# MoFHeka/MeepoEmbedding

Hardware: AMD Instinct MI355X
Metric: key-lookups/sec (higher is better)
Workload: dtype int64 keys / fp32 rows (copy)

## Files before the change

### meepoembedding_amd/csrc/meepo_router.hip

```cpp
#include <hip/hip_runtime.h>

#include <cstdlib>
#include <cstring>
#include <new>

#include "meepo_device.h"
#include "meepo_host.h"

struct mee_router {
    int device;
    uint64_t max_batch;
    uint32_t n_shards;
    uint32_t max_blocks;
    uint32_t* blockcnt;
    uint64_t* base;
    uint64_t* run_base;
    uint64_t* run_sums;
};

struct mee_p2p {
    int device;
    uint32_t n_shards, rank, dim;
    uint64_t cap, max_batch;
    int64_t* inbox_keys;
    int32_t* inbox_dst;
    uint32_t* inbox_cnt;
    float* out;
    uint8_t* found;
    float* inbox_rows;
    uint32_t* status;
    void** d_tables;
    void* h_tables[6][64];
    bool connected;
};

namespace mee {

constexpr int kPartBlock = 1024;
constexpr int kMaxShards = 64;
constexpr uint32_t kNoOwner = 0xFFFFFFFFu;

template <class T>
__device__ __forceinline__ T wave_scan_inclusive(T v, int lane) {
#pragma unroll
    for (int d = 1; d < 64; d <<= 1) {
        const T t = __shfl_up(v, d);
        if (lane >= d) v += t;
    }
    return v;
}

template <bool RANK>
__device__ __forceinline__ uint32_t count_owners(uint32_t o, uint32_t g, uint32_t (&wcnt)[kPartBlock / 64][kMaxShards]) {
    const int lane = threadIdx.x & 63, w = threadIdx.x >> 6;
    uint32_t r = 0;
    for (uint32_t p = 0; p < g; ++p) {
        const uint64_t m = __ballot(o == p);
        if (RANK && o == p) r = (uint32_t)__popcll(m & ((1ull << lane) - 1));
        if (lane == 0) wcnt[w][p] = (uint32_t)__popcll(m);
    }
    __syncthreads();
    if (RANK && o != kNoOwner)
        for (int ww = 0; ww < w; ++ww) r += wcnt[ww][o];
    return r;
}
__device__ __forceinline__ void store_block_counts(const uint32_t (&wcnt)[kPartBlock / 64][kMaxShards], uint32_t g, uint32_t* blockcnt) {
    if (threadIdx.x < g) {
        uint32_t c = 0;
#pragma unroll
        for (int ww = 0; ww < kPartBlock / 64; ++ww) c += wcnt[ww][threadIdx.x];
        blockcnt[(uint64_t)blockIdx.x * g + threadIdx.x] = c;
    }
}

__global__ void hash_batch_kernel(const int64_t* __restrict__ keys, uint64_t n, uint64_t nb, uint32_t g, uint64_t* mix_out,
                                  uint64_t* bucket_out, uint32_t* owner_out) {
    for (uint64_t i = blockIdx.x * (uint64_t)blockDim.x + threadIdx.x; i < n; i += (uint64_t)gridDim.x * blockDim.x) {
        const int64_t k = keys[i];
        if (mix_out) mix_out[i] = mix64((uint64_t)k);
        if (bucket_out) bucket_out[i] = bucket_of(k, nb);
        if (owner_out) owner_out[i] = owner_of(k, g);
    }
}

template <bool SKIP_PAD>
__global__ __launch_bounds__(kPartBlock) void part_count_kernel(const int64_t* __restrict__ keys, uint32_t n, uint32_t g,
                                                                uint32_t* blockcnt) {
    __shared__ uint32_t wcnt[kPartBlock / 64][kMaxShards];
    const uint32_t i = blockIdx.x * kPartBlock + threadIdx.x;
    const int64_t key = i < n ? keys[i] : kEmpty;
    const bool inb = i < n && !(SKIP_PAD && key == kEmpty);
    count_owners<false>(inb ? owner_of(key, g) : kNoOwner, g, wcnt);
    store_block_counts(wcnt, g, blockcnt);
}

__global__ __launch_bounds__(1024) void part_scan_kernel(uint32_t* blockcnt, uint32_t n_blocks, uint32_t g, uint64_t* base,
                                                         uint64_t* counts_out) {
    __shared__ uint64_t total[kMaxShards];
    const int lane = threadIdx.x & 63, w = threadIdx.x >> 6, nw = blockDim.x >> 6;
    for (uint32_t p = w; p < g; p += nw) {
        uint32_t run = 0;
        for (uint32_t b0 = 0; b0 < n_blocks; b0 += 64) {
            const uint32_t b = b0 + lane;
            const uint32_t c = b < n_blocks ? blockcnt[(uint64_t)b * g + p] : 0;
            const uint32_t incl = wave_scan_inclusive(c, lane);
            if (b < n_blocks) blockcnt[(uint64_t)b * g + p] = run + incl - c;
            run += __shfl(incl, 63);
        }
        if (lane == 0) total[p] = run;
    }
    __syncthreads();
    if (threadIdx.x == 0) {
        uint64_t acc = 0;
        for (uint32_t p = 0; p < g; ++p) {
            base[p] = acc;
            counts_out[p] = total[p];
            acc += total[p];
        }
    }
}

template <bool SKIP_PAD>
__global__ __launch_bounds__(kPartBlock) void part_scatter_kernel(const int64_t* __restrict__ keys, uint32_t n, uint32_t g,
                                                                  const uint32_t* __restrict__ blockoff,
                                                                  const uint64_t* __restrict__ base, int64_t* send_keys,
                                                                  int64_t* perm) {
    __shared__ uint32_t wcnt[kPartBlock / 64][kMaxShards];
    const uint32_t i = blockIdx.x * kPartBlock + threadIdx.x;
    const int64_t key = i < n ? keys[i] : kEmpty;
    const bool inb = i < n && !(SKIP_PAD && key == kEmpty);
    const uint32_t o = inb ? owner_of(key, g) : kNoOwner;
    const uint32_t r = count_owners<true>(o, g, wcnt);
    if (inb) {
        const uint64_t dst = base[o] + blockoff[(uint64_t)blockIdx.x * g + o] + r;
        send_keys[dst] = key;
        perm[dst] = (int64_t)i;
    }
}

template <typename T, bool SCATTER>
__global__ void permute_rows_kernel(const T* __restrict__ rows, const int64_t* __restrict__ perm, uint64_t n, uint32_t epr,
                                    T* __restrict__ out) {
    const uint64_t total = n * epr;
    for (uint64_t idx = blockIdx.x * (uint64_t)blockDim.x + threadIdx.x; idx < total; idx += (uint64_t)gridDim.x * blockDim.x) {
        const uint64_t q = idx / epr;
        const uint32_t e = (uint32_t)(idx - q * epr);
        const uint64_t p = (uint64_t)perm[q];
        if (SCATTER) out[p * epr + e] = rows[idx];
        else out[idx] = rows[p * epr + e];
    }
}

template <bool SCATTER>
static int permute_rows(const void* d_rows, const int64_t* d_perm, size_t n, size_t row_bytes, void* d_out, void* stream,
                        const char* name) {
    if (n && (!d_rows || !d_perm || !d_out)) return fail(MEE_ERR_INVALID_ARG, "%s: null argument", name);
    if (n == 0 || row_bytes == 0) return MEE_OK;
    hipStream_t st = (hipStream_t)stream;
    const bool a16 = row_bytes % 16 == 0 && ((uintptr_t)d_rows % 16 == 0) && ((uintptr_t)d_out % 16 == 0);
    const bool a4 = row_bytes % 4 == 0 && ((uintptr_t)d_rows % 4 == 0) && ((uintptr_t)d_out % 4 == 0);
    if (a16) {
        const uint32_t epr = (uint32_t)(row_bytes / 16);
        permute_rows_kernel<float4, SCATTER><<<grid_for(n * epr, 256, 1u << 16), 256, 0, st>>>((const float4*)d_rows, d_perm, n, epr, (float4*)d_out);
    } else if (a4) {
        const uint32_t epr = (uint32_t)(row_bytes / 4);
        permute_rows_kernel<uint32_t, SCATTER><<<grid_for(n * epr, 256, 1u << 16), 256, 0, st>>>((const uint32_t*)d_rows, d_perm, n, epr, (uint32_t*)d_out);
    } else {
        const uint32_t epr = (uint32_t)row_bytes;
        permute_rows_kernel<uint8_t, SCATTER><<<grid_for(n * epr, 256, 1u << 16), 256, 0, st>>>((const uint8_t*)d_rows, d_perm, n, epr, (uint8_t*)d_out);
    }
    MEE_HIP(hipGetLastError());
    return MEE_OK;
}

__device__ __forceinline__ uint32_t last_not_above(const uint64_t* __restrict__ off, uint32_t m, uint64_t i) {
    uint32_t lo = 0, hi = m - 1;
    while (lo < hi) {
        const uint32_t mid = lo + (hi - lo + 1) / 2;
        if (off[mid] <= i) lo = mid; else hi = mid - 1;
    }
    return lo;
}

struct RunPos {
    bool head;
    uint32_t seg;
    uint32_t bag;
    uint32_t seg_end;
};

__device__ __forceinline__ RunPos run_position(const int64_t* __restrict__ perm, const uint64_t* __restrict__ counts, uint32_t g, uint32_t n,
                                               const uint64_t* __restrict__ off, uint32_t n_bags, uint32_t* s_end, uint32_t* s_bag) {
    if (threadIdx.x == 0) {
        uint64_t acc = 0;
        for (uint32_t p = 0; p < g; ++p) {
            const uint64_t c = counts[p];
            acc += c < n ? c : n;
            acc = acc < n ? acc : n;
            s_end[p] = (uint32_t)acc;
        }
    }
    __syncthreads();
    const uint32_t q = blockIdx.x * kPartBlock + threadIdx.x;
    const bool inb = q < s_end[g - 1];
    uint32_t seg = 0;
    while (seg + 1 < g && s_end[seg] <= q) ++seg;
    const uint32_t seg_begin = seg ? s_end[seg - 1] : 0;
    const uint32_t bag = inb ? last_not_above(off, n_bags, (uint64_t)perm[q]) : 0;
    s_bag[threadIdx.x] = bag;
    __syncthreads();
    uint32_t prev = 0;
    if (inb && q > seg_begin) prev = threadIdx.x ? s_bag[threadIdx.x - 1] : last_not_above(off, n_bags, (uint64_t)perm[q - 1]);
    RunPos r;
    r.head = inb && (q == seg_begin || bag != prev);
    r.seg = r.head ? seg : kNoOwner;
    r.bag = bag;
    r.seg_end = s_end[seg];
    return r;
}

__global__ __launch_bounds__(kPartBlock) void run_count_kernel(const int64_t* __restrict__ perm, const uint64_t* __restrict__ counts, uint32_t g, uint32_t n,
                                                              const uint64_t* __restrict__ off, uint32_t n_bags, uint32_t* blockcnt) {
    __shared__ uint32_t s_end[kMaxShards], s_bag[kPartBlock], wcnt[kPartBlock / 64][kMaxShards];
    const RunPos r = run_position(perm, counts, g, n, off, n_bags, s_end, s_bag);
    count_owners<false>(r.seg, g, wcnt);
    store_block_counts(wcnt, g, blockcnt);
}

__global__ __launch_bounds__(kPartBlock) void run_scatter_kernel(const int64_t* __restrict__ perm, const uint64_t* __restrict__ counts, uint32_t g, uint32_t n,
                                                                const uint64_t* __restrict__ off, uint32_t n_bags, const uint32_t* __restrict__ blockoff,
                                                                const uint64_t* __restrict__ run_base, uint32_t* __restrict__ run_bag,
                                                                uint32_t* __restrict__ run_len) {
    __shared__ uint32_t s_end[kMaxShards], s_bag[kPartBlock], wcnt[kPartBlock / 64][kMaxShards];
    const RunPos r = run_position(perm, counts, g, n, off, n_bags, s_end, s_bag);
    const uint32_t rank = count_owners<true>(r.seg, g, wcnt);
    if (r.head) {
        const uint64_t dst = run_base[r.seg] + blockoff[(uint64_t)blockIdx.x * g + r.seg] + rank;
        const uint32_t q = blockIdx.x * kPartBlock + threadIdx.x;
        const uint64_t bag_end = off[r.bag + 1];
        uint32_t lo = q + 1, hi = r.seg_end;
        while (lo < hi) {
            const uint32_t mid = lo + (hi - lo) / 2;
            if ((uint64_t)perm[mid] < bag_end) lo = mid + 1; else hi = mid;
        }
        run_bag[dst] = r.bag;
        run_len[dst] = lo - q;
    }
}

__device__ __forceinline__ uint64_t block_scan_exclusive(uint64_t v, uint64_t* s_w, uint64_t& total) {
    const int lane = threadIdx.x & 63, w = threadIdx.x >> 6, nw = blockDim.x >> 6;
    const uint64_t incl = wave_scan_inclusive(v, lane);
    if (lane == 63) s_w[w] = incl;
    __syncthreads();
    uint64_t before = 0;
    total = 0;
    for (int ww = 0; ww < nw; ++ww) {
        if (ww < w) before += s_w[ww];
        total += s_w[ww];
    }
    __syncthreads();
    return before + incl - v;
}

__global__ __launch_bounds__(kPartBlock) void run_len_sum_kernel(const uint32_t* __restrict__ run_len, uint64_t n_runs, uint64_t* __restrict__ sums) {
    __shared__ uint64_t s_w[kPartBlock / 64];
    const uint64_t i = (uint64_t)blockIdx.x * kPartBlock + threadIdx.x;
    uint64_t total;
    (void)block_scan_exclusive(i < n_runs ? run_len[i] : 0, s_w, total);
    if (threadIdx.x == 0) sums[blockIdx.x] = total;
}

__global__ __launch_bounds__(kPartBlock) void run_len_scan_kernel(uint64_t* sums, uint32_t n_blocks) {
    __shared__ uint64_t s_w[kPartBlock / 64];
    uint64_t carry = 0;
    for (uint32_t b0 = 0; b0 < n_blocks; b0 += kPartBlock) {
        const uint32_t b = b0 + threadIdx.x;
        uint64_t total;
        const uint64_t ex = block_scan_exclusive(b < n_blocks ? sums[b] : 0, s_w, total);
        if (b < n_blocks) sums[b] = carry + ex;
        carry += total;
    }
}

__global__ __launch_bounds__(kPartBlock) void run_offsets_kernel(const uint32_t* __restrict__ run_len, uint64_t n_runs, const uint64_t* __restrict__ sums,
                                                                uint64_t* __restrict__ offsets) {
    __shared__ uint64_t s_w[kPartBlock / 64];
    const uint64_t i = (uint64_t)blockIdx.x * kPartBlock + threadIdx.x;
    const uint64_t len = i < n_runs ? run_len[i] : 0;
    uint64_t total;
    const uint64_t ex = sums[blockIdx.x] + block_scan_exclusive(len, s_w, total);
    if (i < n_runs) offsets[i] = ex;
    if (i + 1 == n_runs) offsets[n_runs] = ex + len;
}

__global__ void run_of_key_kernel(const uint64_t* __restrict__ offsets, uint32_t n_runs, uint64_t n_keys, uint32_t* __restrict__ run_of_key) {
    for (uint64_t k = blockIdx.x * (uint64_t)blockDim.x + threadIdx.x; k < n_keys; k += (uint64_t)gridDim.x * blockDim.x)
        run_of_key[k] = last_not_above(offsets, n_runs, k);
}

template <int DIM4, bool BF16>
__global__ __launch_bounds__(256) void combine_bag_runs_kernel(const float4* __restrict__ partials, const uint32_t* __restrict__ run_bag,
                                                               const uint64_t* __restrict__ run_counts, uint32_t g, uint64_t n_runs,
                                                               const uint64_t* __restrict__ bag_offsets, uint64_t n_bags, uint32_t dim4_rt, int mean,
                                                               void* __restrict__ out) {
    const int lane = threadIdx.x & 63, tile = lane >> 4, tl = lane & 15;
    const uint64_t wave = (uint64_t)blockIdx.x * (blockDim.x >> 6) + (threadIdx.x >> 6);
    const uint64_t n_waves = (uint64_t)gridDim.x * (blockDim.x >> 6);
    const uint32_t dim4 = DIM4 ? DIM4 : dim4_rt;
    const uint64_t seg_c = (uint32_t)lane < g ? run_counts[lane] : 0;
    const uint64_t seg_incl = wave_scan_inclusive(seg_c < n_runs ? seg_c : n_runs, lane);
    const uint64_t seg_hi = seg_incl < n_runs ? seg_incl : n_runs;
    const uint64_t seg_lo_all = __shfl_up(seg_hi, 1);
    const uint64_t seg_lo = lane ? seg_lo_all : 0;
    for (uint64_t b0 = wave * 4; b0 < n_bags; b0 += n_waves * 4) {
        const uint64_t bag = b0 + tile;
        const bool has = bag < n_bags;
        const uint64_t begin = has ? bag_offsets[bag] : 0, end = has ? bag_offsets[bag + 1] : 0;
        const float len = end > begin ? (float)(end - begin) : 0.f;
        int64_t mine[kMaxShards / 16];
#pragma unroll
        for (int k = 0; k < kMaxShards / 16; ++k) {
            mine[k] = -1;
            if ((uint32_t)k * 16 >= g) continue;
            const uint32_t p = (uint32_t)k * 16 + tl;
            uint64_t lo = __shfl(seg_lo, (int)p), hi = __shfl(seg_hi, (int)p);
            if (p >= g || !has) hi = lo;
            const uint64_t stop = hi;
            while (lo < hi) {
                const uint64_t mid = lo + (hi - lo) / 2;
                if (run_bag[mid] < bag) lo = mid + 1; else hi = mid;
            }
            if (lo < stop && run_bag[lo] == bag) mine[k] = (int64_t)lo;
        }
        for (uint32_t c0 = 0; c0 < dim4; c0 += 16) {
            const uint32_t c = c0 + tl;
            const bool col = DIM4 != 0 || c < dim4;
            float4 acc = make_float4(0.f, 0.f, 0.f, 0.f);
            bool first = true;
#pragma unroll
            for (int k = 0; k < kMaxShards / 16; ++k) {
                if ((uint32_t)k * 16 >= g) continue;
#pragma unroll
                for (int j0 = 0; j0 < 16; j0 += 4) {
                    int64_t r[4];
                    float4 row[4];
#pragma unroll
                    for (int u = 0; u < 4; ++u) r[u] = __shfl(mine[k], tile * 16 + j0 + u);
#pragma unroll
                    for (int u = 0; u < 4; ++u) row[u] = (r[u] >= 0 && col) ? partials[(uint64_t)r[u] * dim4 + c] : make_float4(0.f, 0.f, 0.f, 0.f);
#pragma unroll
                    for (int u = 0; u < 4; ++u) {
                        if (r[u] < 0) continue;
                        if (first) acc = row[u];
                        else { acc.x += row[u].x; acc.y += row[u].y; acc.z += row[u].z; acc.w += row[u].w; }
                        first = false;
                    }
                }
            }
            if (has && col) {
                if (mean && !first && len > 0.f) { acc.x = acc.x / len; acc.y = acc.y / len; acc.z = acc.z / len; acc.w = acc.w / len; }
                if constexpr (BF16) store_bf16x4<true>(out, bag * dim4 + c, acc);
                else reinterpret_cast<float4*>(out)[bag * dim4 + c] = acc;
            }
        }
    }
}

__global__ __launch_bounds__(256) void segment_counts_kernel(const int64_t* __restrict__ perm, const uint64_t* __restrict__ counts, uint32_t n,
                                                            const uint64_t* __restrict__ offsets, uint32_t n_tables, uint64_t* __restrict__ cells) {
    __shared__ uint32_t s_bound[257];
    const uint32_t p = blockIdx.x, j0 = blockIdx.y * 256;
    uint64_t acc = 0;
    uint32_t seg_begin = 0;
    for (uint32_t pp = 0; pp <= p; ++pp) {
        seg_begin = (uint32_t)acc;
        const uint64_t c = counts[pp];
        acc += c < n ? c : n;
        acc = acc < n ? acc : n;
    }
    const uint32_t seg_end = (uint32_t)acc;
    for (uint32_t k = threadIdx.x; k < 257; k += 256) {
        const uint32_t j = j0 + k;
        if (j > n_tables) continue;
        const uint64_t bound = offsets[j];
        uint32_t lo = seg_begin, hi = seg_end;
        while (lo < hi) {
            const uint32_t mid = lo + (hi - lo) / 2;
            if ((uint64_t)perm[mid] < bound) lo = mid + 1; else hi = mid;
        }
        s_bound[k] = lo;
    }
    __syncthreads();
    const uint32_t j = j0 + threadIdx.x;
    if (j < n_tables) {
        const uint32_t b = s_bound[threadIdx.x], e = s_bound[threadIdx.x + 1];
        cells[(uint64_t)p * n_tables + j] = e > b ? e - b : 0;
    }
}
// ... 105 lines not shown
        dd[j] = (int32_t)perm[b0 + j];
    }
    if (pad)
        for (uint64_t j = take + blockIdx.x * (uint64_t)blockDim.x + threadIdx.x; j < cap; j += (uint64_t)gridDim.x * blockDim.x) dk[j] = kEmpty;
    if (blockIdx.x == 0 && threadIdx.x == 0) {
        peers.cnt[p][me] = (uint32_t)take;
        if (cnt > cap) atomicOr(status, 1u);
    }
}

__global__ __launch_bounds__(64) void p2p_barrier_kernel(P2PPeers peers, uint32_t me, uint32_t n_shards, uint32_t* status,
                                                         unsigned long long timeout_ticks) {
    const uint32_t q = threadIdx.x;
    uint32_t epoch = 0;
    if (q == 0) { epoch = status[1] + 1; status[1] = epoch; }
    epoch = __shfl(epoch, 0);
    if (q < n_shards) {
        uint32_t* theirs = peers.cnt[q] + n_shards + me;
        __hip_atomic_store(theirs, epoch, __ATOMIC_RELEASE, __HIP_MEMORY_SCOPE_SYSTEM);
        const uint32_t* mine = peers.cnt[me] + n_shards + q;
        const unsigned long long t0 = wall_clock64();
        while ((int32_t)(__hip_atomic_load(mine, __ATOMIC_ACQUIRE, __HIP_MEMORY_SCOPE_SYSTEM) - epoch) < 0) {
            if (wall_clock64() - t0 > timeout_ticks) { atomicOr(status, 2u); break; }
            __builtin_amdgcn_s_sleep(8);
        }
    }
}

__global__ __launch_bounds__(256) void p2p_push_rows_kernel(const float4* __restrict__ rows, const int64_t* __restrict__ perm,
                                                            const uint64_t* __restrict__ counts, const uint64_t* __restrict__ base,
                                                            P2PPeers peers, uint32_t me, uint64_t cap, uint32_t dim4) {
    const int lane = threadIdx.x & 63, tile = lane >> 4, tl = lane & 15;
    const uint32_t p = blockIdx.y;
    const uint64_t cnt = counts[p];
    const uint64_t take = cnt < cap ? cnt : cap;
    float4* __restrict__ dr = reinterpret_cast<float4*>(peers.rows[p]) + (uint64_t)me * cap * dim4;
    const uint64_t b0 = base[p];
    const uint64_t wave = (uint64_t)blockIdx.x * (blockDim.x >> 6) + (threadIdx.x >> 6), n_waves = (uint64_t)gridDim.x * (blockDim.x >> 6);
    for (uint64_t j0 = wave * 4; j0 < take; j0 += n_waves * 4) {
        const uint64_t j = j0 + tile;
        if (j >= take) continue;
        const uint64_t src = (uint64_t)perm[b0 + j] * dim4;
        for (uint32_t c = tl; c < dim4; c += 16) dr[j * dim4 + c] = rows[src + c];
    }
}

template <int DIM4, int R>
__global__ __launch_bounds__(256) void p2p_find_kernel(const int64_t* __restrict__ tkeys, const float4* __restrict__ values, uint64_t nb,
                                                       uint32_t dim4_rt, float defv, const int64_t* __restrict__ in_keys,
                                                       const int32_t* __restrict__ in_dst, const uint32_t* __restrict__ in_cnt,
                                                       P2PPeers peers, uint64_t cap) {
    const int lane = threadIdx.x & 63, tile = lane >> 4, tl = lane & 15;
    const uint32_t s = blockIdx.y;
    const uint32_t cnt = in_cnt[s];
    const uint32_t wave = blockIdx.x * (blockDim.x >> 6) + (threadIdx.x >> 6);
    const uint32_t n_waves = gridDim.x * (blockDim.x >> 6);
    const int64_t* __restrict__ seg_keys = in_keys + (uint64_t)s * cap;
    const int32_t* __restrict__ seg_dst = in_dst + (uint64_t)s * cap;
    float4* __restrict__ outp = reinterpret_cast<float4*>(peers.out[s]);
    uint8_t* __restrict__ fnd = peers.found[s];
    const uint32_t dim4 = DIM4 ? DIM4 : dim4_rt;
    const float4 def4 = make_float4(defv, defv, defv, defv);
    for (uint32_t base = wave * 4 * R; base < cnt; base += n_waves * 4 * R) {
        int64_t key[R], slot[R];
        int32_t dst[R];
        bool inb[R];
#pragma unroll
        for (int r = 0; r < R; ++r) {
            const uint32_t i = base + r * 4 + tile;
            inb[r] = i < cnt;
            key[r] = inb[r] ? seg_keys[i] : kEmpty;
            dst[r] = inb[r] ? seg_dst[i] : 0;
        }
        uint64_t b[R];
        int64_t kb[R];
#pragma unroll
        for (int r = 0; r < R; ++r) {
            b[r] = bucket_of(key[r], nb);
            kb[r] = (inb[r] && !reserved_key(key[r])) ? tkeys[b[r] * kW + tl] : kEmpty;
        }
#pragma unroll
        for (int r = 0; r < R; ++r) slot[r] = tile_probe(tkeys, nb, key[r], inb[r] && !reserved_key(key[r]), b[r], kb[r], tile, tl);
        if constexpr (DIM4 != 0) {
            constexpr int C = DIM4 / 16;
            float4 row[R][C];
#pragma unroll
            for (int r = 0; r < R; ++r)
#pragma unroll
                for (int c = 0; c < C; ++c) row[r][c] = slot[r] >= 0 ? values[(uint64_t)slot[r] * DIM4 + c * 16 + tl] : def4;
#pragma unroll
            for (int r = 0; r < R; ++r)
                if (inb[r]) {
#pragma unroll
                    for (int c = 0; c < C; ++c) outp[(uint64_t)dst[r] * DIM4 + c * 16 + tl] = row[r][c];
                }
        } else {
#pragma unroll
            for (int r = 0; r < R; ++r)
                if (inb[r])
                    for (uint32_t c = tl; c < dim4; c += 16)
                        outp[(uint64_t)dst[r] * dim4 + c] = slot[r] >= 0 ? values[(uint64_t)slot[r] * dim4 + c] : def4;
        }
#pragma unroll
        for (int r = 0; r < R; ++r)
            if (inb[r] && tl == 0) fnd[dst[r]] = slot[r] >= 0;
    }
}

}

using namespace mee;

extern "C" {

int mee_hash_batch(const int64_t* d_keys, size_t n, uint64_t n_buckets, uint32_t n_shards, uint64_t* d_mix_out,
                   uint64_t* d_bucket_out, uint32_t* d_owner_out, void* stream) {
    MEE_RANGE("mee_hash_batch");
    if (n && !d_keys) return fail(MEE_ERR_INVALID_ARG, "mee_hash_batch: null keys");
    if (n == 0) return MEE_OK;
    hash_batch_kernel<<<grid_for(n, 256, 1u << 14), 256, 0, (hipStream_t)stream>>>(d_keys, n, n_buckets, n_shards, d_mix_out,
                                                                                 d_bucket_out, d_owner_out);
    MEE_HIP(hipGetLastError());
    return MEE_OK;
}

int mee_router_destroy(mee_router* r) {
    MEE_RANGE("mee_router_destroy");
    if (!r) return MEE_OK;
    DeviceGuard g(r->device);
    if (r->blockcnt) (void)hipFree(r->blockcnt);
    if (r->base) (void)hipFree(r->base);
    if (r->run_base) (void)hipFree(r->run_base);
    if (r->run_sums) (void)hipFree(r->run_sums);
    delete r;
    return MEE_OK;
}

int mee_router_create(int32_t device, uint64_t max_batch, uint32_t n_shards, mee_router** out) {
    MEE_RANGE("mee_router_create");
    if (!out) return fail(MEE_ERR_INVALID_ARG, "mee_router_create: null out");
    *out = nullptr;
    if (n_shards == 0 || n_shards > (uint32_t)kMaxShards || max_batch == 0 || max_batch > (1ull << 30))
        return fail(MEE_ERR_INVALID_ARG, "mee_router_create: n_shards must be 1..%d and max_batch 1..2^30", kMaxShards);
    int ndev = 0;
    if (hipGetDeviceCount(&ndev) != hipSuccess || ndev <= 0)
        return fail(MEE_ERR_NO_DEVICE, "mee_router_create: no HIP device visible (this backend has no CPU fallback)");
    if (device < 0 || device >= ndev) return fail(MEE_ERR_INVALID_ARG, "mee_router_create: device %d out of range", device);
    DeviceGuard g(device);
    mee_router* r = new (std::nothrow) mee_router();
    if (!r) return fail(MEE_ERR_OUT_OF_MEMORY, "host allocation failed");
    r->device = device; r->max_batch = max_batch; r->n_shards = n_shards;
    r->max_blocks = (uint32_t)((max_batch + kPartBlock - 1) / kPartBlock);
    r->blockcnt = nullptr; r->base = nullptr; r->run_base = nullptr; r->run_sums = nullptr;
    if (hipMalloc((void**)&r->blockcnt, (size_t)r->max_blocks * n_shards * 4) != hipSuccess ||
        hipMalloc((void**)&r->base, n_shards * 8) != hipSuccess || hipMalloc((void**)&r->run_base, n_shards * 8) != hipSuccess ||
        hipMalloc((void**)&r->run_sums, ((size_t)r->max_blocks * n_shards + 1) * 8) != hipSuccess) {
        mee_router_destroy(r);
        return fail(MEE_ERR_OUT_OF_MEMORY, "mee_router_create: hipMalloc failed");
    }
    *out = r;
    return MEE_OK;
}

static int partition_common(mee_router* r, const int64_t* d_keys, size_t n, int64_t* d_send_keys, uint64_t* d_counts, int64_t* d_perm,
                            void* stream, bool skip_pad, const char* name) {
    if (!r || !d_counts || (n && (!d_keys || !d_send_keys || !d_perm))) return fail(MEE_ERR_INVALID_ARG, "%s: null argument", name);
    if (n > r->max_batch) return fail(MEE_ERR_BATCH_TOO_LARGE, "%s: n=%zu exceeds max_batch=%llu", name, n, (unsigned long long)r->max_batch);
    DeviceGuard g(r->device);
    hipStream_t st = (hipStream_t)stream;
    const uint32_t nblk = (uint32_t)((n + kPartBlock - 1) / kPartBlock);
    if (nblk) with_flag(skip_pad, [&](auto sp) { part_count_kernel<sp><<<nblk, kPartBlock, 0, st>>>(d_keys, (uint32_t)n, r->n_shards, r->blockcnt); });
    part_scan_kernel<<<1, 1024, 0, st>>>(r->blockcnt, nblk, r->n_shards, r->base, d_counts);
    if (nblk) with_flag(skip_pad, [&](auto sp) { part_scatter_kernel<sp><<<nblk, kPartBlock, 0, st>>>(d_keys, (uint32_t)n, r->n_shards, r->blockcnt, r->base, d_send_keys, d_perm); });
    MEE_HIP(hipGetLastError());
    return MEE_OK;
}
int mee_partition(mee_router* r, const int64_t* d_keys, size_t n, int64_t* d_send_keys, uint64_t* d_counts, int64_t* d_perm,
                  void* stream) {
    MEE_RANGE("mee_partition");
    return partition_common(r, d_keys, n, d_send_keys, d_counts, d_perm, stream, false, "mee_partition");
}
int mee_partition_padded(mee_router* r, const int64_t* d_keys, size_t n, int64_t* d_send_keys, uint64_t* d_counts, int64_t* d_perm,
                         void* stream) {
    MEE_RANGE("mee_partition_padded");
    return partition_common(r, d_keys, n, d_send_keys, d_counts, d_perm, stream, true, "mee_partition_padded");
}

int mee_bag_runs(mee_router* r, const int64_t* d_perm, const uint64_t* d_counts, size_t n, const uint64_t* d_bag_offsets, size_t n_bags,
                 uint32_t* d_run_bag, uint32_t* d_run_len, uint64_t* d_run_counts, void* stream) {
    MEE_RANGE("mee_bag_runs");
    if (!r || !d_counts || !d_bag_offsets || !d_run_counts || (n && (!d_perm || !d_run_bag || !d_run_len)))
        return fail(MEE_ERR_INVALID_ARG, "mee_bag_runs: null argument");
    if (n > r->max_batch) return fail(MEE_ERR_BATCH_TOO_LARGE, "mee_bag_runs: n=%zu exceeds max_batch=%llu", n, (unsigned long long)r->max_batch);
    if (n_bags > 0xFFFFFFFFull || (n && n_bags == 0)) return fail(MEE_ERR_INVALID_ARG, "mee_bag_runs: n_bags must be in [1, 2^32) when there are positions (the bags partition them)");
    DeviceGuard g(r->device);
    hipStream_t st = (hipStream_t)stream;
    const uint32_t nblk = (uint32_t)((n + kPartBlock - 1) / kPartBlock);
    if (nblk) run_count_kernel<<<nblk, kPartBlock, 0, st>>>(d_perm, d_counts, r->n_shards, (uint32_t)n, d_bag_offsets, (uint32_t)n_bags, r->blockcnt);
    part_scan_kernel<<<1, 1024, 0, st>>>(r->blockcnt, nblk, r->n_shards, r->run_base, d_run_counts);
    if (nblk) run_scatter_kernel<<<nblk, kPartBlock, 0, st>>>(d_perm, d_counts, r->n_shards, (uint32_t)n, d_bag_offsets, (uint32_t)n_bags, r->blockcnt, r->run_base, d_run_bag, d_run_len);
    MEE_HIP(hipGetLastError());
    return MEE_OK;
}

int mee_run_offsets(mee_router* r, const uint32_t* d_run_len, size_t n_runs, uint64_t* d_offsets, uint32_t* d_run_of_key, size_t n_keys, void* stream) {
    MEE_RANGE("mee_run_offsets");
    if (!r || !d_offsets || (n_runs && !d_run_len)) return fail(MEE_ERR_INVALID_ARG, "mee_run_offsets: null argument");
    if (n_runs > (size_t)r->max_batch * r->n_shards)
        return fail(MEE_ERR_BATCH_TOO_LARGE, "mee_run_offsets: n_runs=%zu exceeds n_shards x max_batch=%llu", n_runs, (unsigned long long)(r->max_batch * r->n_shards));
    if (n_runs > 0xFFFFFFFFull) return fail(MEE_ERR_BATCH_TOO_LARGE, "mee_run_offsets: n_runs=%zu does not fit the 32-bit run index", n_runs);
    if (d_run_of_key && n_keys && n_runs == 0) return fail(MEE_ERR_INVALID_ARG, "mee_run_offsets: %zu keys but no run", n_keys);
    DeviceGuard g(r->device);
    hipStream_t st = (hipStream_t)stream;
    if (n_runs == 0) {
        MEE_HIP(hipMemsetAsync(d_offsets, 0, 8, st));
        return MEE_OK;
    }
    const uint32_t nblk = (uint32_t)((n_runs + kPartBlock - 1) / kPartBlock);
    run_len_sum_kernel<<<nblk, kPartBlock, 0, st>>>(d_run_len, n_runs, r->run_sums);
    run_len_scan_kernel<<<1, kPartBlock, 0, st>>>(r->run_sums, nblk);
    run_offsets_kernel<<<nblk, kPartBlock, 0, st>>>(d_run_len, n_runs, r->run_sums, d_offsets);
    if (d_run_of_key && n_keys) run_of_key_kernel<<<grid_for(n_keys, 256, 1u << 16), 256, 0, st>>>(d_offsets, (uint32_t)n_runs, n_keys, d_run_of_key);
    MEE_HIP(hipGetLastError());
    return MEE_OK;
}

int mee_combine_bag_runs(mee_router* r, const float* d_partials, const uint32_t* d_run_bag, const uint64_t* d_run_counts, size_t n_runs,
                         const uint64_t* d_bag_offsets, size_t n_bags, uint32_t dim, int mode, void* d_out, uint32_t out_dtype, void* stream) {
    MEE_RANGE("mee_combine_bag_runs");
    if (!r || !d_run_counts || (n_bags && (!d_bag_offsets || !d_out)) || (n_runs && (!d_partials || !d_run_bag)))
        return fail(MEE_ERR_INVALID_ARG, "mee_combine_bag_runs: null argument");
    if (int rc = check_out_dtype(d_out, out_dtype, "mee_combine_bag_runs")) return rc;
    if (mode != MEE_POOL_SUM && mode != MEE_POOL_MEAN) return fail(MEE_ERR_INVALID_ARG, "mee_combine_bag_runs: mode must be MEE_POOL_SUM or MEE_POOL_MEAN");
    if (dim < 4 || (dim & 3) || ((uintptr_t)d_partials & 15) || (out_dtype == MEE_DTYPE_F32 && ((uintptr_t)d_out & 15)))
        return fail(MEE_ERR_INVALID_ARG, "mee_combine_bag_runs: dim must be a positive multiple of 4 and fp32 rows 16-byte aligned");
    if (n_runs > 0xFFFFFFFFull) return fail(MEE_ERR_BATCH_TOO_LARGE, "mee_combine_bag_runs: n_runs=%zu", n_runs);
    if (n_bags == 0) return MEE_OK;
    DeviceGuard g(r->device);
    hipStream_t st = (hipStream_t)stream;
    with_row_shape(dim / 4, [&](auto d4) { with_flag(out_dtype == MEE_DTYPE_BF16, [&](auto bf16) {
        combine_bag_runs_kernel<d4, bf16><<<grid_for(n_bags, 16, 1u << 20), 256, 0, st>>>((const float4*)d_partials, d_run_bag, d_run_counts, r->n_shards, n_runs,
                                                                                         d_bag_offsets, n_bags, dim / 4, mode == MEE_POOL_MEAN, d_out);
    }); });
    MEE_HIP(hipGetLastError());
    return MEE_OK;
}

int mee_segment_counts(mee_router* r, const int64_t* d_perm, const uint64_t* d_counts, size_t n, const uint64_t* d_offsets, size_t n_tables,
                       uint64_t* d_cell_counts, void* stream) {
    MEE_RANGE("mee_segment_counts");
    if (!r || !d_counts || !d_offsets || !d_cell_counts || (n && !d_perm)) return fail(MEE_ERR_INVALID_ARG, "mee_segment_counts: null argument");
    if (n > r->max_batch) return fail(MEE_ERR_BATCH_TOO_LARGE, "mee_segment_counts: n=%zu exceeds max_batch=%llu", n, (unsigned long long)r->max_batch);
    if (n_tables == 0 || n_tables > kMaxGroupTables) return fail(MEE_ERR_INVALID_ARG, "mee_segment_counts: n_tables must be in [1, %u]", kMaxGroupTables);
    DeviceGuard g(r->device);
    const dim3 grid(r->n_shards, (unsigned)((n_tables + 255) / 256));
    segment_counts_kernel<<<grid, 256, 0, (hipStream_t)stream>>>(d_perm, d_counts, (uint32_t)n, d_offsets, (uint32_t)n_tables, d_cell_counts);
    MEE_HIP(hipGetLastError());
    return MEE_OK;
}

int mee_regroup(mee_router* r, const int64_t* d_recv_keys, const uint64_t* d_recv_cells, size_t n_recv, size_t n_tables, int64_t* d_keys_out,
                int64_t* d_order_out, uint64_t* d_offsets_out, void* stream) {
    MEE_RANGE("mee_regroup");
    if (!r || !d_recv_cells || !d_offsets_out || (n_recv && (!d_recv_keys || !d_keys_out || !d_order_out))) return fail(MEE_ERR_INVALID_ARG, "mee_regroup: null argument");
    if (n_recv > (size_t)r->max_batch * r->n_shards)
        return fail(MEE_ERR_BATCH_TOO_LARGE, "mee_regroup: n_recv=%zu exceeds n_shards x max_batch=%llu", n_recv, (unsigned long long)(r->max_batch * r->n_shards));
    if (n_recv > 0xFFFFFFFFull - 2 * kPartBlock) return fail(MEE_ERR_BATCH_TOO_LARGE, "mee_regroup: n_recv=%zu does not fit the 32-bit position", n_recv);
    if (n_tables == 0 || n_tables > kMaxGroupTables || n_tables * r->n_shards > (size_t)kRegroupMaxCells)
        return fail(MEE_ERR_INVALID_ARG, "mee_regroup: n_tables must be in [1, %u] and n_shards x n_tables <= %d (the cell offsets live in LDS)", kMaxGroupTables, kRegroupMaxCells);
    DeviceGuard g(r->device);
    const size_t lds = 2 * (n_tables * r->n_shards + 1) * sizeof(uint32_t);
    const bool a16 = (((uintptr_t)d_recv_keys | (uintptr_t)d_keys_out | (uintptr_t)d_order_out) & 15) == 0;
    with_flag(a16, [&](auto wide) {
        constexpr int V = decltype(wide)::value ? 2 : 1;
        regroup_kernel<V><<<grid_for(n_recv, kRegroupBlock * V, 1u << 23), kRegroupBlock, lds, (hipStream_t)stream>>>(
            d_recv_keys, d_recv_cells, (uint32_t)n_recv, r->n_shards, (uint32_t)n_tables, d_keys_out, d_order_out, d_offsets_out);
    });
    MEE_HIP(hipGetLastError());
    return MEE_OK;
}

int mee_p2p_destroy(mee_p2p* c) {
    MEE_RANGE("mee_p2p_destroy");
    if (!c) return MEE_OK;
    DeviceGuard g(c->device);
    (void)hipDeviceSynchronize();
    if (c->connected)
        for (int b = 0; b < kP2PBuffers; ++b)
            for (uint32_t p = 0; p < c->n_shards; ++p)
                if (p != c->rank && c->h_tables[b][p]) (void)hipIpcCloseMemHandle(c->h_tables[b][p]);
    void* mine[] = {c->inbox_keys, c->inbox_dst, c->inbox_cnt, c->out, c->found, c->inbox_rows, c->status, c->d_tables};
    for (void* p : mine) if (p) (void)hipFree(p);
    delete c;
    return MEE_OK;
}

int mee_p2p_create(int32_t device, uint32_t n_shards, uint32_t rank, uint64_t slots_per_peer, uint64_t max_batch, uint32_t dim,
                   int with_payload, mee_p2p** out) {
    MEE_RANGE("mee_p2p_create");
    if (!out) return fail(MEE_ERR_INVALID_ARG, "mee_p2p_create: null out");
    *out = nullptr;
    if (n_shards == 0 || n_shards > (uint32_t)kMaxShards || rank >= n_shards || slots_per_peer == 0 || max_batch == 0 ||
        max_batch > (1ull << 30) || dim < 4 || (dim & 3))
        return fail(MEE_ERR_INVALID_ARG, "mee_p2p_create: bad arguments");
    int ndev = 0;
    if (hipGetDeviceCount(&ndev) != hipSuccess || ndev <= 0) return fail(MEE_ERR_NO_DEVICE, "mee_p2p_create: no HIP device visible");
    if (device < 0 || device >= ndev) return fail(MEE_ERR_INVALID_ARG, "mee_p2p_create: device %d out of range", device);
    DeviceGuard g(device);
    mee_p2p* c = new (std::nothrow) mee_p2p();
    if (!c) return fail(MEE_ERR_OUT_OF_MEMORY, "host allocation failed");
    memset(c, 0, sizeof *c);
    c->device = device; c->n_shards = n_shards; c->rank = rank; c->dim = dim; c->cap = slots_per_peer; c->max_batch = max_batch;
    const uint64_t slots = (uint64_t)n_shards * slots_per_peer;
    const bool fine = getenv("MEE_P2P_COARSE") == nullptr;
    auto sym_alloc = [&](void** p, size_t bytes) {
        return fine ? hipExtMallocWithFlags(p, bytes, hipDeviceMallocFinegrained) : hipMalloc(p, bytes);
    };
    if (sym_alloc((void**)&c->inbox_keys, slots * 8) != hipSuccess || sym_alloc((void**)&c->inbox_dst, slots * 4) != hipSuccess ||
        sym_alloc((void**)&c->inbox_cnt, 2 * n_shards * 4) != hipSuccess || sym_alloc((void**)&c->out, (max_batch + 1) * (uint64_t)dim * 4) != hipSuccess ||
        sym_alloc((void**)&c->found, max_batch + 1) != hipSuccess ||
        (with_payload && sym_alloc((void**)&c->inbox_rows, slots * (uint64_t)dim * 4) != hipSuccess) ||
        hipMalloc((void**)&c->status, 8) != hipSuccess ||
        hipMalloc((void**)&c->d_tables, kP2PBuffers * (size_t)n_shards * sizeof(void*)) != hipSuccess) {
        mee_p2p_destroy(c);
        return fail(MEE_ERR_OUT_OF_MEMORY, "mee_p2p_create: device allocation failed (%s)", fine ? "fine-grained" : "coarse-grained");
    }
    if (hipMemset(c->inbox_cnt, 0, 2 * n_shards * 4) != hipSuccess || hipMemset(c->status, 0, 8) != hipSuccess) {
        mee_p2p_destroy(c);
        return fail(MEE_ERR_HIP, "mee_p2p_create: hipMemset failed");
    }
    *out = c;
    return MEE_OK;
}

static void* p2p_local(const mee_p2p* c, int b) {
    switch (b) { case 0: return c->inbox_keys; case 1: return c->inbox_dst; case 2: return c->inbox_cnt; case 3: return c->out; case 4: return c->found; default: return c->inbox_rows; }
}

int mee_p2p_export(mee_p2p* c, void* handles) {
    MEE_RANGE("mee_p2p_export");
    if (!c || !handles) return fail(MEE_ERR_INVALID_ARG, "mee_p2p_export: null argument");
    static_assert(sizeof(hipIpcMemHandle_t) == MEE_IPC_HANDLE_BYTES, "IPC handle size");
    DeviceGuard g(c->device);
    memset(handles, 0, (size_t)kP2PBuffers * MEE_IPC_HANDLE_BYTES);
    for (int b = 0; b < kP2PBuffers; ++b) {
        if (!p2p_local(c, b)) continue;
        hipIpcMemHandle_t h;
        MEE_HIP(hipIpcGetMemHandle(&h, p2p_local(c, b)));
        memcpy((char*)handles + b * MEE_IPC_HANDLE_BYTES, &h, MEE_IPC_HANDLE_BYTES);
    }
    return MEE_OK;
}

// ... 124 lines not shown
```

Before: 7.887 billion.

## Replace three-kernel partition with sliced count+scatter and in-block scan

Partition and bag-run routing now process up to 256 fixed slices per kernel, each block looping over several 1024-key tiles with double-buffered shared counters and prefetch of the next key. The separate single-block scan kernel is removed; each scatter block recomputes its per-shard start offsets from the small blockcnt table. This saves a kernel launch and the serial single-block scan, and shrinks blockcnt traffic. In exchange, each block runs a longer serial loop and repeats a small redundant reduction, and fewer blocks may leave CUs idle on small batches.

After: 7.876 billion. No clear change (-0.1%).

```diff
diff --git a/meepoembedding_amd/csrc/meepo_router.hip b/meepoembedding_amd/csrc/meepo_router.hip
--- a/meepoembedding_amd/csrc/meepo_router.hip
+++ b/meepoembedding_amd/csrc/meepo_router.hip
@@ -37,6 +37,7 @@
 namespace mee {
 
 constexpr int kPartBlock = 1024;
+constexpr int kPartRows = 256;
 constexpr int kMaxShards = 64;
 constexpr uint32_t kNoOwner = 0xFFFFFFFFu;
 
@@ -64,12 +65,56 @@
         for (int ww = 0; ww < w; ++ww) r += wcnt[ww][o];
     return r;
 }
-__device__ __forceinline__ void store_block_counts(const uint32_t (&wcnt)[kPartBlock / 64][kMaxShards], uint32_t g, uint32_t* blockcnt) {
-    if (threadIdx.x < g) {
-        uint32_t c = 0;
-#pragma unroll
-        for (int ww = 0; ww < kPartBlock / 64; ++ww) c += wcnt[ww][threadIdx.x];
-        blockcnt[(uint64_t)blockIdx.x * g + threadIdx.x] = c;
+__device__ __forceinline__ uint32_t step_count(const uint32_t (&wcnt)[kPartBlock / 64][kMaxShards], uint32_t p) {
+    uint32_t c = 0;
+#pragma unroll
+    for (int ww = 0; ww < kPartBlock / 64; ++ww) c += wcnt[ww][p];
+    return c;
+}
+
+struct PartSlices { uint32_t n_blocks, slice; };
+static PartSlices part_slices(size_t n) {
+    size_t s = (n + kPartRows - 1) / kPartRows;
+    s = (s + kPartBlock - 1) / kPartBlock * kPartBlock;
+    if (s < (size_t)kPartBlock) s = kPartBlock;
+    return {(uint32_t)((n + s - 1) / s), (uint32_t)s};
+}
+
+__device__ __forceinline__ void block_starts(const uint32_t* __restrict__ blockcnt, uint32_t n_blocks, uint32_t g, uint32_t* s_tot, uint32_t* s_bef,
+                                             uint32_t* s_run, uint64_t* base_out, uint64_t* counts_out) {
+    const uint32_t lane = threadIdx.x & 63, w = threadIdx.x >> 6;
+    if (threadIdx.x < kMaxShards) { s_tot[threadIdx.x] = 0; s_bef[threadIdx.x] = 0; }
+    __syncthreads();
+    const uint32_t rpl = 64 / g;
+    const uint32_t p = lane % g, sub = lane / g;
+    const uint32_t stride = (kPartBlock / 64) * rpl;
+    uint32_t tot = 0, bef = 0;
+    for (uint32_t row0 = w * rpl + sub; row0 - sub < n_blocks; row0 += 4 * stride) {
+        uint32_t c[4];
+#pragma unroll
+        for (int u = 0; u < 4; ++u) {
+            const uint32_t row = row0 + u * stride;
+            c[u] = blockcnt[sub < rpl && row < n_blocks ? row * g + p : 0];
+        }
+#pragma unroll
+        for (int u = 0; u < 4; ++u) {
+            const uint32_t row = row0 + u * stride;
+            if (sub < rpl && row < n_blocks) {
+                tot += c[u];
+                if (row < blockIdx.x) bef += c[u];
+            }
+        }
+    }
+    if (tot) atomicAdd(&s_tot[p], tot);
+    if (bef) atomicAdd(&s_bef[p], bef);
+    __syncthreads();
+    if (w == 0) {
+        const uint32_t c = lane < g ? s_tot[lane] : 0;
+        const uint32_t first = wave_scan_inclusive(c, (int)lane) - c;
+        if (lane < g) {
+            s_run[lane] = first + s_bef[lane];
+            if (blockIdx.x == 0) { base_out[lane] = first; counts_out[lane] = c; }
+        }
     }
 }
 
@@ -84,57 +129,47 @@
 }
 
 template <bool SKIP_PAD>
-__global__ __launch_bounds__(kPartBlock) void part_count_kernel(const int64_t* __restrict__ keys, uint32_t n, uint32_t g,
+__global__ __launch_bounds__(kPartBlock) void part_count_kernel(const int64_t* __restrict__ keys, uint32_t n, uint32_t slice, uint32_t g,
                                                                 uint32_t* blockcnt) {
-    __shared__ uint32_t wcnt[kPartBlock / 64][kMaxShards];
-    const uint32_t i = blockIdx.x * kPartBlock + threadIdx.x;
-    const int64_t key = i < n ? keys[i] : kEmpty;
-    const bool inb = i < n && !(SKIP_PAD && key == kEmpty);
-    count_owners<false>(inb ? owner_of(key, g) : kNoOwner, g, wcnt);
-    store_block_counts(wcnt, g, blockcnt);
-}
-
-__global__ __launch_bounds__(1024) void part_scan_kernel(uint32_t* blockcnt, uint32_t n_blocks, uint32_t g, uint64_t* base,
-                                                         uint64_t* counts_out) {
-    __shared__ uint64_t total[kMaxShards];
-    const int lane = threadIdx.x & 63, w = threadIdx.x >> 6, nw = blockDim.x >> 6;
-    for (uint32_t p = w; p < g; p += nw) {
-        uint32_t run = 0;
-        for (uint32_t b0 = 0; b0 < n_blocks; b0 += 64) {
-            const uint32_t b = b0 + lane;
-            const uint32_t c = b < n_blocks ? blockcnt[(uint64_t)b * g + p] : 0;
-            const uint32_t incl = wave_scan_inclusive(c, lane);
-            if (b < n_blocks) blockcnt[(uint64_t)b * g + p] = run + incl - c;
-            run += __shfl(incl, 63);
-        }
-        if (lane == 0) total[p] = run;
-    }
-    __syncthreads();
-    if (threadIdx.x == 0) {
-        uint64_t acc = 0;
-        for (uint32_t p = 0; p < g; ++p) {
-            base[p] = acc;
-            counts_out[p] = total[p];
-            acc += total[p];
-        }
-    }
+    __shared__ uint32_t wcnt[2][kPartBlock / 64][kMaxShards];
+    const uint32_t first = blockIdx.x * slice, end = first + slice < n ? first + slice : n;
+    int64_t key = first + threadIdx.x < end ? keys[first + threadIdx.x] : kEmpty;
+    uint32_t c = 0, buf = 0;
+    for (uint32_t i0 = first; i0 < end; i0 += kPartBlock, buf ^= 1) {
+        const uint32_t i = i0 + threadIdx.x, in = i + kPartBlock;
+        const uint32_t own = owner_of(key, g);
+        const int64_t next = keys[in < end ? in : first];
+        const bool inb = i < end && !(SKIP_PAD && key == kEmpty);
+        count_owners<false>(inb ? own : kNoOwner, g, wcnt[buf]);
+        if (threadIdx.x < g) c += step_count(wcnt[buf], threadIdx.x);
+        key = next;
+    }
+    if (threadIdx.x < g) blockcnt[blockIdx.x * g + threadIdx.x] = c;
 }
 
 template <bool SKIP_PAD>
-__global__ __launch_bounds__(kPartBlock) void part_scatter_kernel(const int64_t* __restrict__ keys, uint32_t n, uint32_t g,
-                                                                  const uint32_t* __restrict__ blockoff,
-                                                                  const uint64_t* __restrict__ base, int64_t* send_keys,
-                                                                  int64_t* perm) {
-    __shared__ uint32_t wcnt[kPartBlock / 64][kMaxShards];
-    const uint32_t i = blockIdx.x * kPartBlock + threadIdx.x;
-    const int64_t key = i < n ? keys[i] : kEmpty;
-    const bool inb = i < n && !(SKIP_PAD && key == kEmpty);
-    const uint32_t o = inb ? owner_of(key, g) : kNoOwner;
-    const uint32_t r = count_owners<true>(o, g, wcnt);
-    if (inb) {
-        const uint64_t dst = base[o] + blockoff[(uint64_t)blockIdx.x * g + o] + r;
-        send_keys[dst] = key;
-        perm[dst] = (int64_t)i;
+__global__ __launch_bounds__(kPartBlock) void part_scatter_kernel(const int64_t* __restrict__ keys, uint32_t n, uint32_t slice, uint32_t g,
+                                                                  const uint32_t* __restrict__ blockcnt, uint32_t n_blocks, uint64_t* base,
+                                                                  uint64_t* counts_out, int64_t* send_keys, int64_t* perm) {
+    __shared__ uint32_t wcnt[2][kPartBlock / 64][kMaxShards], s_tot[kMaxShards], s_bef[kMaxShards], s_run[2][kMaxShards];
+    const uint32_t first = blockIdx.x * slice, end = first + slice < n ? first + slice : n;
+    int64_t key = first + threadIdx.x < end ? keys[first + threadIdx.x] : kEmpty;
+    block_starts(blockcnt, n_blocks, g, s_tot, s_bef, s_run[0], base, counts_out);
+    uint32_t buf = 0;
+    for (uint32_t i0 = first; i0 < end; i0 += kPartBlock, buf ^= 1) {
+        const uint32_t i = i0 + threadIdx.x, in = i + kPartBlock;
+        const uint32_t own = owner_of(key, g);
+        const int64_t next = keys[in < end ? in : first];
+        const bool inb = i < end && !(SKIP_PAD && key == kEmpty);
+        const uint32_t o = inb ? own : kNoOwner;
+        const uint32_t r = count_owners<true>(o, g, wcnt[buf]);
+        if (inb) {
+            const uint32_t dst = s_run[buf][o] + r;
+            send_keys[dst] = key;
+            perm[dst] = (int64_t)i;
+        }
+        if (threadIdx.x < g) s_run[buf ^ 1][threadIdx.x] = s_run[buf][threadIdx.x] + step_count(wcnt[buf], threadIdx.x);
+        key = next;
     }
 }
 
@@ -189,8 +224,7 @@
     uint32_t seg_end;
 };
 
-__device__ __forceinline__ RunPos run_position(const int64_t* __restrict__ perm, const uint64_t* __restrict__ counts, uint32_t g, uint32_t n,
-                                               const uint64_t* __restrict__ off, uint32_t n_bags, uint32_t* s_end, uint32_t* s_bag) {
+__device__ __forceinline__ void segment_ends(const uint64_t* __restrict__ counts, uint32_t g, uint32_t n, uint32_t* s_end) {
     if (threadIdx.x == 0) {
         uint64_t acc = 0;
         for (uint32_t p = 0; p < g; ++p) {
@@ -200,13 +234,14 @@
             s_end[p] = (uint32_t)acc;
         }
     }
-    __syncthreads();
-    const uint32_t q = blockIdx.x * kPartBlock + threadIdx.x;
-    const bool inb = q < s_end[g - 1];
+}
+
+__device__ __forceinline__ RunPos run_position(const int64_t* __restrict__ perm, uint32_t q, bool inb, int64_t pq, uint32_t g, const uint64_t* __restrict__ off,
+                                               uint32_t n_bags, const uint32_t* s_end, uint32_t* s_bag) {
     uint32_t seg = 0;
     while (seg + 1 < g && s_end[seg] <= q) ++seg;
     const uint32_t seg_begin = seg ? s_end[seg - 1] : 0;
-    const uint32_t bag = inb ? last_not_above(off, n_bags, (uint64_t)perm[q]) : 0;
+    const uint32_t bag = inb ? last_not_above(off, n_bags, (uint64_t)pq) : 0;
     s_bag[threadIdx.x] = bag;
     __syncthreads();
     uint32_t prev = 0;
@@ -220,31 +255,52 @@
 }
 
 __global__ __launch_bounds__(kPartBlock) void run_count_kernel(const int64_t* __restrict__ perm, const uint64_t* __restrict__ counts, uint32_t g, uint32_t n,
-                                                              const uint64_t* __restrict__ off, uint32_t n_bags, uint32_t* blockcnt) {
-    __shared__ uint32_t s_end[kMaxShards], s_bag[kPartBlock], wcnt[kPartBlock / 64][kMaxShards];
-    const RunPos r = run_position(perm, counts, g, n, off, n_bags, s_end, s_bag);
-    count_owners<false>(r.seg, g, wcnt);
-    store_block_counts(wcnt, g, blockcnt);
+                                                              uint32_t slice, const uint64_t* __restrict__ off, uint32_t n_bags, uint32_t* blockcnt) {
+    __shared__ uint32_t s_end[kMaxShards], s_bag[kPartBlock], wcnt[2][kPartBlock / 64][kMaxShards];
+    segment_ends(counts, g, n, s_end);
+    __syncthreads();
+    const uint32_t first = blockIdx.x * slice, stop = s_end[g - 1], end = first + slice < stop ? first + slice : stop;
+    int64_t pq = first + threadIdx.x < end ? perm[first + threadIdx.x] : 0;
+    uint32_t c = 0, buf = 0;
+    for (uint32_t q0 = first; q0 < end; q0 += kPartBlock, buf ^= 1) {
+        const uint32_t q = q0 + threadIdx.x, qn = q + kPartBlock;
+        const RunPos r = run_position(perm, q, q < end, pq, g, off, n_bags, s_end, s_bag);
+        const int64_t next = perm[qn < end ? qn : first];
+        count_owners<false>(r.seg, g, wcnt[buf]);
+        if (threadIdx.x < g) c += step_count(wcnt[buf], threadIdx.x);
+        pq = next;
+    }
+    if (threadIdx.x < g) blockcnt[blockIdx.x * g + threadIdx.x] = c;
 }
 
 __global__ __launch_bounds__(kPartBlock) void run_scatter_kernel(const int64_t* __restrict__ perm, const uint64_t* __restrict__ counts, uint32_t g, uint32_t n,
-                                                                const uint64_t* __restrict__ off, uint32_t n_bags, const uint32_t* __restrict__ blockoff,
-                                                                const uint64_t* __restrict__ run_base, uint32_t* __restrict__ run_bag,
-                                                                uint32_t* __restrict__ run_len) {
-    __shared__ uint32_t s_end[kMaxShards], s_bag[kPartBlock], wcnt[kPartBlock / 64][kMaxShards];
-    const RunPos r = run_position(perm, counts, g, n, off, n_bags, s_end, s_bag);
-    const uint32_t rank = count_owners<true>(r.seg, g, wcnt);
-    if (r.head) {
-        const uint64_t dst = run_base[r.seg] + blockoff[(uint64_t)blockIdx.x * g + r.seg] + rank;
-        const uint32_t q = blockIdx.x * kPartBlock + threadIdx.x;
-        const uint64_t bag_end = off[r.bag + 1];
-        uint32_t lo = q + 1, hi = r.seg_end;
-        while (lo < hi) {
-            const uint32_t mid = lo + (hi - lo) / 2;
-            if ((uint64_t)perm[mid] < bag_end) lo = mid + 1; else hi = mid;
-        }
-        run_bag[dst] = r.bag;
-        run_len[dst] = lo - q;
+                                                                uint32_t slice, const uint64_t* __restrict__ off, uint32_t n_bags,
+                                                                const uint32_t* __restrict__ blockcnt, uint32_t n_blocks, uint64_t* run_base,
+                                                                uint64_t* run_counts, uint32_t* __restrict__ run_bag, uint32_t* __restrict__ run_len) {
+    __shared__ uint32_t s_end[kMaxShards], s_bag[kPartBlock], wcnt[2][kPartBlock / 64][kMaxShards], s_tot[kMaxShards], s_bef[kMaxShards], s_run[2][kMaxShards];
+    segment_ends(counts, g, n, s_end);
+    block_starts(blockcnt, n_blocks, g, s_tot, s_bef, s_run[0], run_base, run_counts);
+    const uint32_t first = blockIdx.x * slice, stop = s_end[g - 1], end = first + slice < stop ? first + slice : stop;
+    int64_t pq = first + threadIdx.x < end ? perm[first + threadIdx.x] : 0;
+    uint32_t buf = 0;
+    for (uint32_t q0 = first; q0 < end; q0 += kPartBlock, buf ^= 1) {
+        const uint32_t q = q0 + threadIdx.x, qn = q + kPartBlock;
+        const RunPos r = run_position(perm, q, q < end, pq, g, off, n_bags, s_end, s_bag);
+        const int64_t next = perm[qn < end ? qn : first];
+        const uint32_t rank = count_owners<true>(r.seg, g, wcnt[buf]);
+        if (r.head) {
+            const uint32_t dst = s_run[buf][r.seg] + rank;
+            const uint64_t bag_end = off[r.bag + 1];
+            uint32_t lo = q + 1, hi = r.seg_end;
+            while (lo < hi) {
+                const uint32_t mid = lo + (hi - lo) / 2;
+                if ((uint64_t)perm[mid] < bag_end) lo = mid + 1; else hi = mid;
+            }
+            run_bag[dst] = r.bag;
+            run_len[dst] = lo - q;
+        }
+        if (threadIdx.x < g) s_run[buf ^ 1][threadIdx.x] = s_run[buf][threadIdx.x] + step_count(wcnt[buf], threadIdx.x);
+        pq = next;
     }
 }
 
@@ -656,7 +712,7 @@
     r->device = device; r->max_batch = max_batch; r->n_shards = n_shards;
     r->max_blocks = (uint32_t)((max_batch + kPartBlock - 1) / kPartBlock);
     r->blockcnt = nullptr; r->base = nullptr; r->run_base = nullptr; r->run_sums = nullptr;
-    if (hipMalloc((void**)&r->blockcnt, (size_t)r->max_blocks * n_shards * 4) != hipSuccess ||
+    if (hipMalloc((void**)&r->blockcnt, (size_t)kPartRows * n_shards * 4) != hipSuccess ||
         hipMalloc((void**)&r->base, n_shards * 8) != hipSuccess || hipMalloc((void**)&r->run_base, n_shards * 8) != hipSuccess ||
         hipMalloc((void**)&r->run_sums, ((size_t)r->max_blocks * n_shards + 1) * 8) != hipSuccess) {
         mee_router_destroy(r);
@@ -672,10 +728,12 @@
     if (n > r->max_batch) return fail(MEE_ERR_BATCH_TOO_LARGE, "%s: n=%zu exceeds max_batch=%llu", name, n, (unsigned long long)r->max_batch);
     DeviceGuard g(r->device);
     hipStream_t st = (hipStream_t)stream;
-    const uint32_t nblk = (uint32_t)((n + kPartBlock - 1) / kPartBlock);
-    if (nblk) with_flag(skip_pad, [&](auto sp) { part_count_kernel<sp><<<nblk, kPartBlock, 0, st>>>(d_keys, (uint32_t)n, r->n_shards, r->blockcnt); });
-    part_scan_kernel<<<1, 1024, 0, st>>>(r->blockcnt, nblk, r->n_shards, r->base, d_counts);
-    if (nblk) with_flag(skip_pad, [&](auto sp) { part_scatter_kernel<sp><<<nblk, kPartBlock, 0, st>>>(d_keys, (uint32_t)n, r->n_shards, r->blockcnt, r->base, d_send_keys, d_perm); });
+    const PartSlices ps = part_slices(n);
+    with_flag(skip_pad, [&](auto sp) {
+        if (ps.n_blocks) part_count_kernel<sp><<<ps.n_blocks, kPartBlock, 0, st>>>(d_keys, (uint32_t)n, ps.slice, r->n_shards, r->blockcnt);
+        part_scatter_kernel<sp><<<ps.n_blocks ? ps.n_blocks : 1, kPartBlock, 0, st>>>(d_keys, (uint32_t)n, ps.slice, r->n_shards, r->blockcnt, ps.n_blocks, r->base,
+                                                                                    d_counts, d_send_keys, d_perm);
+    });
     MEE_HIP(hipGetLastError());
     return MEE_OK;
 }
@@ -699,10 +757,10 @@
     if (n_bags > 0xFFFFFFFFull || (n && n_bags == 0)) return fail(MEE_ERR_INVALID_ARG, "mee_bag_runs: n_bags must be in [1, 2^32) when there are positions (the bags partition them)");
     DeviceGuard g(r->device);
     hipStream_t st = (hipStream_t)stream;
-    const uint32_t nblk = (uint32_t)((n + kPartBlock - 1) / kPartBlock);
-    if (nblk) run_count_kernel<<<nblk, kPartBlock, 0, st>>>(d_perm, d_counts, r->n_shards, (uint32_t)n, d_bag_offsets, (uint32_t)n_bags, r->blockcnt);
-    part_scan_kernel<<<1, 1024, 0, st>>>(r->blockcnt, nblk, r->n_shards, r->run_base, d_run_counts);
-    if (nblk) run_scatter_kernel<<<nblk, kPartBlock, 0, st>>>(d_perm, d_counts, r->n_shards, (uint32_t)n, d_bag_offsets, (uint32_t)n_bags, r->blockcnt, r->run_base, d_run_bag, d_run_len);
+    const PartSlices ps = part_slices(n);
+    if (ps.n_blocks) run_count_kernel<<<ps.n_blocks, kPartBlock, 0, st>>>(d_perm, d_counts, r->n_shards, (uint32_t)n, ps.slice, d_bag_offsets, (uint32_t)n_bags, r->blockcnt);
+    run_scatter_kernel<<<ps.n_blocks ? ps.n_blocks : 1, kPartBlock, 0, st>>>(d_perm, d_counts, r->n_shards, (uint32_t)n, ps.slice, d_bag_offsets, (uint32_t)n_bags, r->blockcnt,
+                                                                             ps.n_blocks, r->run_base, d_run_counts, d_run_bag, d_run_len);
     MEE_HIP(hipGetLastError());
     return MEE_OK;
 }
```
